# themeshpotato/rust-ray-tracing-in-a-weekend

Measured on AMD Instinct MI355X. Metric: Msamples/s (pixels x spp) for 1200x800 random-spheres scene, higher is better.
Workload: dtype f64

## Files before the change

include/rt/rt_abi.h:

```cpp
#ifndef RT_ABI_H
#define RT_ABI_H

#include <stddef.h>
#include <stdint.h>

#include "rt_scene.h"

#ifdef __cplusplus
extern "C" {
#endif

#define RT_ABI_VERSION 6

enum {
    RT_OK = 0,
    RT_ERR_INVALID = -1,
    RT_ERR_HIP = -2,
    RT_ERR_UNSUPPORTED = -3,
    RT_ERR_OOM = -4,
    RT_ERR_NO_DEVICE = -5,
    RT_ERR_NO_SCENE = -6,
    RT_ERR_COMM = -7,
    RT_ERR_PEER = -8
};
// ... 125 lines not shown
    uint64_t wave_leaf_steps;
    uint64_t camera_lanes;
    uint64_t camera_steps;
    uint64_t shade_lanes;
    uint64_t shade_steps;
    int32_t precision;
    int32_t waves_per_simd;
    int64_t trace_buf_bytes;
    int32_t overlapped;
    int32_t reserved0;
    int64_t ring_bytes;
    int64_t primary_table_bytes;
    double primary_build_ms;
    double primary_walk_share;
    int64_t sky_tiles;
} rt_stats;
int rt_last_stats(rt_ctx* ctx, rt_stats* out);

typedef struct rt_primary_candidates_info {
    int64_t pixels, flagged;
    int64_t candidates;
    int32_t max_candidates;
    int32_t slots;
} rt_primary_candidates_info;
int rt_primary_candidates_host(const rt_scene_soa* scene, const rt_camera* cam, int width, int height, int k_max,
                               uint16_t* records, rt_primary_candidates_info* info);
int rt_primary_sky_tiles_host(const rt_scene_soa* scene, const rt_camera* cam, int width, int height, int k_max,
                              uint8_t* flags, int64_t* count);
int rt_last_counters(rt_ctx* ctx, uint64_t* out, int n);

// ... 308 lines not shown

int rt_ctx_set_variant(rt_ctx* ctx, int slab32, int lds_stack, int lds_nodes);

enum {
    RT_OPT_TRACE_BUF_BYTES = 1,
    RT_OPT_BATCH_OVERLAP = 2,
    RT_OPT_BLOCK_SAMPLES = 3,
    RT_OPT_BLOCK_CHUNKS = 4,
    RT_OPT_EXTRA_FEATURES = 5,
    RT_OPT_HOIST = 6,
    RT_OPT_POOL_RING = 9,
    RT_OPT_COMM_DIRECT = 10,
    RT_OPT_AUTO_DEAL_ORDER = 11,
    RT_OPT_PRIMARY_CANDIDATES = 12,
    RT_OPT_PRIMARY_CANDIDATES_K = 13,
    RT_OPT_SKIP_SKY_TILES = 14
};
int rt_ctx_set_option(rt_ctx* ctx, int key, int64_t value);
int rt_ctx_get_option(rt_ctx* ctx, int key, int64_t* value);

enum { RT_SCHED_CHUNKS = 0, RT_SCHED_POOL = 1, RT_SCHED_ITEMS = 2, RT_SCHED_AUTO = 3 };
int rt_ctx_set_schedule(rt_ctx* ctx, int schedule);

enum { RT_PREC_F64 = 0, RT_PREC_F32 = 1 };
int rt_ctx_set_precision(rt_ctx* ctx, int precision);

int rt_device_eval(rt_ctx* ctx, int fn, const double* x, const double* y, const double* z, double* out, int n);

#ifdef __cplusplus
}
#endif
// ... 2 lines not shown
```

rust-ray-tracing-in-a-weekend_amd/csrc/abi.cpp:

```cpp
#include <hip/hip_runtime.h>

#include <algorithm>
#include <cmath>
#include <cstring>
#include <new>
#include <string>
#include <vector>

#include "rt/rt_abi.h"
#include "rt/rt_numerics.h"
#include "camera_rays.hpp"
#include "ctx_internal.hpp"
#include "deal_cache.hpp"
#include "launch_plan.hpp"
#include "primary_candidates.hpp"
#include "render_internal.hpp"
#include "scene_lower.hpp"
#include "trace_kernel.hpp"

namespace {

thread_local std::string g_last_error;

}
// ... 317 lines not shown
    }
    if (sky) {
        *dealt_tiles = img_tiles - c->sky_n;
        c->stats.sky_tiles = c->sky_n;
    }
    return RT_OK;
}

static int primary_setup(rt_ctx* c, const rt_camera* cam, const rt_render_params* p, const rtp::Plan& pl, bool count_work,
                         hipStream_t stream, rtk::KParams& K, rtk::LaunchOpts& o)
{
    rt_stats& st = c->stats;
    st.primary_table_bytes = 0;
    st.primary_build_ms = 0.0;
    st.primary_walk_share = 0.0;
    const size_t bytes = rtpc::table_bytes(p->width, p->height);
    if (!c->opt_primary || pl.variant != rtk::FEAT_SET_SPHERES || pl.f32 || pl.schedule != RT_SCHED_POOL || !pl.shape.s16 ||
        pl.seed_stage_bytes == 0 || count_work || bytes > rtpc::kMaxTableBytes || p->width < 2 || p->height < 2)
        return RT_OK;
    rtd::Key key = rtd::key_of(c->upload_gen, *cam, *p);
    key.row_begin = 0;
    key.row_stride = key.row_block = 1;
    if (!(c->primary_valid && rtd::same_key(key, c->primary_key) && c->primary_k == c->opt_primary_k)) {
        c->primary_valid = false;
        int rc = c->primary_tab.reserve(stream, bytes + 16);
        if (rc) return rc;
        const size_t n_tiles = (size_t)rtpc::tiles_x_of(p->width) * (size_t)rtpc::tiles_y_of(p->height);
        rc = c->sky_tab.reserve(stream, 16 + n_tiles);
        if (rc) return rc;
        unsigned* const flagged = reinterpret_cast<unsigned*>(c->primary_tab.as<char>() + bytes);
// ... 7 lines not shown
        HIP_TRY(hipMemcpyAsync(&n_sky, c->sky_tab.p, sizeof n_sky, hipMemcpyDeviceToHost, stream));
        HIP_TRY(hipMemcpyAsync(c->sky_flags.data(), c->sky_dev(), n_tiles, hipMemcpyDeviceToHost, stream));
        HIP_TRY(hipStreamSynchronize(stream));
        c->sky_n = (int64_t)n_sky;
        c->sky_gen++;
        float ms = 0.0f;
        HIP_TRY(c->ev_pc.elapsed(0, &ms));
        c->primary_key = key;
        c->primary_k = c->opt_primary_k;
        c->primary_flagged = (int64_t)n_flagged;
        c->primary_valid = true;
        st.primary_build_ms = ms;
    }
    K.primary = c->primary_tab.as<uint4>();
    o.primary = 1;
    st.primary_table_bytes = (int64_t)bytes;
    st.primary_walk_share = (double)c->primary_flagged / ((double)p->width * (double)p->height);
    return RT_OK;
}

static void write_stats(rt_ctx* c, const rtp::Plan& pl, int chunk, int waves_per_simd, bool count)
{
    rt_stats& st = c->stats;
    st.lds_nodes = pl.n_lds_nodes;
    st.variant_features = (int32_t)pl.variant;
    st.slab32 = pl.slab32;
    st.lds_stack = pl.lds_stack;
    st.schedule = pl.schedule;
    st.precision = pl.f32 ? RT_PREC_F32 : RT_PREC_F64;
    st.waves_per_simd = waves_per_simd;
// ... 483 lines not shown
        if (v < 0 || v > 2) return fail(RT_ERR_INVALID, "deal order mode out of range (0 off, 1 auto, 2 measure only)");
        c->opt_deal = (int)v;
        return RT_OK;
    case RT_OPT_PRIMARY_CANDIDATES:
        if (v < 0 || v > 1) return fail(RT_ERR_INVALID, "primary candidates out of range (0 off, 1 on)");
        c->opt_primary = (int)v;
        return RT_OK;
    case RT_OPT_PRIMARY_CANDIDATES_K:
        if (v < 1 || v > rtpc::kSlots) return fail(RT_ERR_INVALID, "primary candidates per pixel out of range (1..7)");
        c->opt_primary_k = (int)v;
        return RT_OK;
    case RT_OPT_SKIP_SKY_TILES:
        if (v < 0 || v > 1) return fail(RT_ERR_INVALID, "skip sky tiles out of range (0 off, 1 on)");
        c->opt_sky = (int)v;
        return RT_OK;
    default: return fail(RT_ERR_INVALID, "unknown option");
    }
}

int rt_ctx_get_option(rt_ctx* c, int key, int64_t* v)
{
    if (!c || !v) return fail(RT_ERR_INVALID, "null argument");
    switch (key) {
    case RT_OPT_TRACE_BUF_BYTES: *v = (int64_t)c->sample_buf_cap; return RT_OK;
    case RT_OPT_BATCH_OVERLAP: *v = c->opt.overlap; return RT_OK;
    case RT_OPT_BLOCK_SAMPLES: *v = c->opt.block_samples; return RT_OK;
    case RT_OPT_BLOCK_CHUNKS: *v = c->opt.block_chunks; return RT_OK;
    case RT_OPT_EXTRA_FEATURES: *v = c->opt.extra_features; return RT_OK;
    case RT_OPT_HOIST: *v = c->opt_hoist; return RT_OK;
    case RT_OPT_POOL_RING: *v = c->opt.ring; return RT_OK;
    case RT_OPT_COMM_DIRECT: *v = c->opt_comm_direct; return RT_OK;
    case RT_OPT_AUTO_DEAL_ORDER: *v = c->opt_deal; return RT_OK;
    case RT_OPT_PRIMARY_CANDIDATES: *v = c->opt_primary; return RT_OK;
    case RT_OPT_PRIMARY_CANDIDATES_K: *v = c->opt_primary_k; return RT_OK;
    case RT_OPT_SKIP_SKY_TILES: *v = c->opt_sky; return RT_OK;
    default: return fail(RT_ERR_INVALID, "unknown option");
    }
}

int rt_ctx_set_schedule(rt_ctx* c, int schedule)
{
    if (c && schedule == 4)
        return fail(RT_ERR_UNSUPPORTED, "schedule 4 (wavefront) was removed: 2.3x slower than the pool on C4 (DESIGN.md 5.7)");
    if (!c || schedule < RT_SCHED_CHUNKS || schedule > RT_SCHED_AUTO) return fail(RT_ERR_INVALID, "bad schedule");
    c->opt.schedule = schedule;
    return RT_OK;
}

int rt_device_eval(rt_ctx* c, int fn, const double* x, const double* y, const double* z, double* out, int n)
{
// ... 19 lines not shown
```

rust-ray-tracing-in-a-weekend_amd/csrc/ctx_internal.hpp:

```cpp
#pragma once

#include <hip/hip_runtime.h>

#include <cstddef>
#include <cstdint>
#include <string>
#include <vector>

#include "rt/rt_abi.h"
#include "deal_cache.hpp"
#include "launch_plan.hpp"
#include "trace_kernel.hpp"

namespace rtx {

int fail(int code, const std::string& msg);
int hip_fail(hipError_t e, const char* what);

}

using rtx::fail;
using rtx::hip_fail;

#define HIP_TRY(expr)                                   \
// ... 147 lines not shown
    DevBuf acc_tmp;
    int opt_deal = rtd::kAuto;
    uint64_t upload_gen = 0;
    rtd::DealCache deal;
    int64_t deal_cap = 0;
    int64_t last_deal_n = 0;
    int opt_primary = 1;
    int opt_primary_k = 7;
    DevBuf primary_tab;
    bool primary_valid = false;
    rtd::Key primary_key;
    int primary_k = 0;
    int64_t primary_flagged = 0;
    EventSpan<2> ev_pc;
    int opt_sky = 1;
    DevBuf sky_tab;
    std::vector<uint8_t> sky_flags;
    int64_t sky_n = 0;
    uint64_t sky_gen = 0;
    uint64_t deal_sky_gen = 0;
    uint8_t* sky_dev() const { return reinterpret_cast<uint8_t*>(sky_tab.p) + 16; }
};

struct StreamScope {
    rt_ctx* c;
    hipStream_t stream;
    bool open = false;
    StreamScope(rt_ctx* c_, hipStream_t s_) : c(c_), stream(s_) {}
    int begin()
    {
// ... 20 lines not shown
```

rust-ray-tracing-in-a-weekend_amd/csrc/trace_kernel.hip:

```cpp
#include "trace_launch.hpp"

namespace rtk {

__device__ __forceinline__ bool tile_slot(SampleTiles g, int n_samples, long long i, long long& px, size_t& rec)
{
    const long long tile = i >> 6;
    const int lp = (int)(i & 63);
    const int x = (int)(tile % g.tiles_x) * 8 + (lp & 7);
    const int k = (int)(tile / g.tiles_x) * 8 + (lp >> 3);
    if (x >= g.width || k >= g.n_rows) return false;
    px = (long long)k * g.width + x;
    rec = tiled_record(g.tiles_x, n_samples, x, k, 0);
    return true;
}

constexpr int kReduceWaves = 8;
template <typename T, typename Rec = double>
__global__ void __launch_bounds__(64 * kReduceWaves) reduce_samples_tiled(const Rec* __restrict__ samples,
                                                                          T* __restrict__ out, SampleTiles g,
                                                                          int n_samples, int chunk, double scale,
                                                                          SkyTiles sky)
{
    __shared__ double part[kReduceWaves][3][64];
    const unsigned tile = blockIdx.x;
// ... 225 lines not shown
}

hipError_t launch_trace(const SceneDev& S, const KParams& Ph, const KParams* P, double* out,
                        unsigned long long* counters, unsigned* work, const LaunchOpts& o, hipStream_t stream)
{
    Launch L;
    L.S = &S;
    L.P = P;
    L.out = out;
    L.counters = counters;
    L.work = work;
    L.pool = o.pool;
    L.waves_per_simd = o.waves_per_simd;
    L.max_waves = o.pool == 1 && Ph.ring ? (unsigned)Ph.ring_waves : 0u;
    L.primary = o.primary != 0 && Ph.primary != nullptr;
    const long long groups = o.pool == 2   ? (Ph.n_chunks + std::max(1, Ph.block_chunks) - 1) / std::max(1, Ph.block_chunks)
                             : o.pool == 1 ? ((long long)Ph.spp - Ph.sample_begin + std::max(1, Ph.block_samples) - 1) /
                                                 std::max(1, Ph.block_samples)
                                           : Ph.n_chunks;
    L.n_blocks = (unsigned long long)Ph.tiles_x * Ph.tiles_y * groups;
    if (L.n_blocks == 0) return hipSuccess;
    if (L.n_blocks > 0xfffffff0ULL) return hipErrorInvalidValue;
    if (o.pool) {
        const hipError_t e = hipMemsetAsync(work, 0, sizeof(unsigned), stream);
        if (e != hipSuccess) return e;
    }
    const uint32_t f = variant_features(o.features);
    if (o.f32) return o.count ? launch_kind<true, true>(f, L, o, stream) : launch_kind<false, true>(f, L, o, stream);
    return o.count ? launch_kind<true, false>(f, L, o, stream) : launch_kind<false, false>(f, L, o, stream);
}
// ... 90 lines not shown
```

rust-ray-tracing-in-a-weekend_amd/csrc/trace_kernel.hpp:

```cpp
#pragma once

#include <hip/hip_runtime.h>

#include "rt/rt_scene.h"
#include "scene_features.hpp"
#include "launch_shapes.hpp"

namespace rtk {

struct SceneDev {
    const rt_prim* prims;
    const int32_t* prim_refs;
    const rt_prim* leaf_prims;
    const rt_bvh_node* nodes;
    const rt_instance* instances;
    const rt_material* materials;
    const rt_texture* textures;
    const double* perlin_ranvec;
    const int32_t* perlin_perm;
    const uint8_t* image;
    int32_t tlas_root;
    int32_t blas_base;
    int32_t stack_entries;
    int32_t n_lds_nodes;
// ... 39 lines not shown
    const uint4* primary;
};

constexpr int32_t kDealOrdered = 2, kDealMeasure = 3;
constexpr unsigned kDealTable = 16;
constexpr bool deal_variant(uint32_t variant) { return variant == FEAT_SET_SPHERES; }

struct LaunchOpts {
    uint32_t features;
    int slab32;
    int lds_stack;
    int count;
    int pool;
    int f32;
    int primary = 0;
    int* waves_per_simd = nullptr;
};

enum CounterSlot : int {
    kCtrCasts = 0,
    kCtrNodeVisits = 1,
    kCtrPrimTests = 2,
    kCtrCyclesCamera = 3,
    kCtrCyclesTrace = 4,
    kCtrCyclesShade = 5,
    kCtrWaveSteps = 6,
    kCtrWaveNodeSteps = 7,
    kCtrCyclesNodes = 8,
    kCtrCyclesLeaves = 9,
    kCtrWaveLeafSteps = 10,
// ... 84 lines not shown
```

rust-ray-tracing-in-a-weekend_amd/csrc/trace_launch.hpp:

```cpp
#pragma once
#include "trace_device.hpp"
#include "trace_launch_common.hpp"

namespace rtk {

template <uint32_t F, bool COUNT, bool F32 = false>
hipError_t launch_variant(const Launch& L, const LaunchOpts& o, hipStream_t stream)
{
    const SceneDev& S = *L.S;
    KernelShape k = launch_shape(F, F32, S, o);
    if constexpr (!F32) {
        if (k.s16) {
            using C = Cfg<F, true, true, true, COUNT, false>;
            static const bool static_lds =
                any_static_lds({(const void*)trace_pool<C, false>, (const void*)trace_pool<C, true>,
                                (const void*)trace_pool<C, false, true>, (const void*)trace_chunks<C>}) ||
                [] {
                    if constexpr (RT_STAGE_SEEDS != 0 && C::SHAPE.s16)
                        return any_static_lds({(const void*)trace_pool<CfgStage<C>, false>, (const void*)trace_pool<CfgStage<C>, false, true>});
                    else return false;
                }() ||
                [] {
                    if constexpr (RT_STAGE_SEEDS != 0 && C::SHAPE.s16 && F == FEAT_SET_SPHERES && !COUNT)
                        return any_static_lds({(const void*)trace_pool<CfgPrimary<C>, false>, (const void*)trace_pool<CfgPrimary<C>, false, true>});
                    else return false;
                }();
            if (static_lds) k = without_stack16(k);
        }
    }
    const int bt = k.block_threads, wpb = bt / 64;
    const int seed_bytes = RT_STAGE_SEEDS && k.s16 && !F32 && L.pool == 1 && S.seed_stage_bytes == (int)seed_stage_bytes_of(bt)
                               ? S.seed_stage_bytes : 0;
    const size_t lds = launch_lds_bytes(k, S, seed_bytes);
    with_cfg<F, COUNT, F32>(k, [&](auto whole, auto part) {
        using C1 = decltype(whole);
        using C0 = decltype(part);
        if (L.pool) {
            auto go = [&](auto kernel) {
                unsigned nb = std::min<unsigned long long>(resident_blocks(L, kernel, lds, bt), (L.n_blocks + wpb - 1) / wpb);
                if (L.max_waves) nb = std::max(1u, std::min(nb, L.max_waves / (unsigned)wpb));
                hipLaunchKernelGGL(kernel, dim3(nb), dim3(bt), lds, stream, S, L.P, L.out, L.counters, L.work);
            };
            if constexpr (RT_STAGE_SEEDS != 0 && C1::SHAPE.s16 && !F32 && F == FEAT_SET_SPHERES && !COUNT) {
                if (seed_bytes && L.primary)
                    return go(L.max_waves ? trace_pool<CfgPrimary<C1>, false, true> : trace_pool<CfgPrimary<C1>, false>);
            }
            if constexpr (RT_STAGE_SEEDS != 0 && C1::SHAPE.s16 && !F32) {
                if (seed_bytes) return go(L.max_waves ? trace_pool<CfgStage<C1>, false, true> : trace_pool<CfgStage<C1>, false>);
            }
            if (L.pool == 2) go(k.nall ? trace_pool<C1, true> : trace_pool<C0, true>);
            else if (L.max_waves)
                go(k.nall ? trace_pool<C1, false, true> : trace_pool<C0, false, true>);
            else go(k.nall ? trace_pool<C1, false> : trace_pool<C0, false>);
            return;
        }
        const auto kernel = k.nall ? trace_chunks<C1> : trace_chunks<C0>;
        if (L.waves_per_simd) (void)blocks_per_cu(L, kernel, lds, bt);
        hipLaunchKernelGGL(kernel, dim3((unsigned)((L.n_blocks + wpb - 1) / wpb)), dim3(bt), lds, stream, S, L.P, L.out, L.counters);
// ... 27 lines not shown
```

rust-ray-tracing-in-a-weekend_amd/csrc/trace_launch_common.hpp:

```cpp
#pragma once
#include "trace_types.hpp"

namespace rtk {

struct Launch {
    const SceneDev* S;
    const KParams* P;
    double* out;
    unsigned long long* counters;
    unsigned* work;
    int pool;
    unsigned long long n_blocks;
    int* waves_per_simd;
    unsigned max_waves = 0;
    bool primary = false;
};

template <class K>
static int blocks_per_cu(const Launch& L, K kernel, size_t lds, int bt)
{
    int per_cu = 0;
    if (hipOccupancyMaxActiveBlocksPerMultiprocessor(&per_cu, kernel, bt, lds) != hipSuccess || per_cu <= 0) per_cu = 1;
    if (L.waves_per_simd) *L.waves_per_simd = per_cu * (bt / 256);
    return per_cu;
}

template <class K>
static unsigned resident_blocks(const Launch& L, K kernel, size_t lds, int bt)
{
    static int cus = 0;
// ... 42 lines not shown
```

rust-ray-tracing-in-a-weekend_amd/csrc/trace_pool.hpp:

```cpp
#pragma once
#include "trace_shade.hpp"
#include "trace_grid.hpp"

namespace rtk {

template <class R>
__device__ __forceinline__ void forget(HitT<R>& h)
{
    h.t = __builtin_nondeterministic_value(h.t);
    h.px = __builtin_nondeterministic_value(h.px);
    h.py = __builtin_nondeterministic_value(h.py);
    h.pz = __builtin_nondeterministic_value(h.pz);
    h.nx = __builtin_nondeterministic_value(h.nx);
    h.ny = __builtin_nondeterministic_value(h.ny);
    h.nz = __builtin_nondeterministic_value(h.nz);
    h.uv0 = __builtin_nondeterministic_value(h.uv0);
    h.uv1 = __builtin_nondeterministic_value(h.uv1);
    h.uv2 = __builtin_nondeterministic_value(h.uv2);
    h.uv3 = __builtin_nondeterministic_value(h.uv3);
    h.front = __builtin_nondeterministic_value(h.front);
    h.mat = __builtin_nondeterministic_value(h.mat);
    h.uvkind = __builtin_nondeterministic_value(h.uvkind);
}

// ... 109 lines not shown
            camera_end(P, st, u, v, qx, qy, r);
            const unsigned n = rec.x & 0xffffu;
            if (n > 7u || depth <= 0) go = true;
            else {
                finish_ray<C, false>(r, true);
                n_cand = n + 1;
            }
        }
        if (__any(n_cand != 0)) {
            const R t_min = (R)0.001;
            R t_max = (R)RT_INF;
            HitRefT<R> best;
            best.sub = 0;
            best.side = 0;
            best.prim = -1;
            uint64_t a = ((uint64_t)rec.y << 32 | (uint64_t)rec.x) >> 16;
            const uint64_t b = (uint64_t)rec.w << 32 | (uint64_t)rec.z;
#pragma unroll 1
            for (unsigned i = 0; __ballot(i + 1 < n_cand) != 0; ++i) {
                if (i + 1 < n_cand) {
                    const int slot = (int)((unsigned)a & 0xffffu);
                    if (simple_t<C>(S.leaf_prims[slot], r, t_min, t_max, best.t, best.side, cnt, false)) {
                        best.prim = slot;
                        t_max = best.t;
                    }
                }
                a >>= 16;
                if (i == 2) a = b;
            }
            if (n_cand != 0) {
                if (best.prim < 0) {
                    cr = cr + Tr * P.bg[0];
                    cg = cg + Tg * P.bg[1];
                    cb = cb + Tb * P.bg[2];
                } else {
                    finish_hit<C>(S, r, best, h);
                    pending = shade_begin<C>(S, h, Tr, Tg, Tb, cr, cg, cb);
                }
            }
        }
    }
    if (__any(pending)) {
        R qx = (R)0, qy = (R)0, qz = (R)0, l2 = (R)1;
        bool accepted = !(pending && shade_draws<C>(S, h.mat));
        for (int n = 1;; ++n) {
            if (!accepted) accepted = unit_try(st, (R)P.scale_m11, true, qx, qy, qz, l2);
            const uint64_t rejecting = __ballot(!accepted);
            if (rejecting == 0 || (n >= RT_TRY_MIN && __popcll(rejecting) <= RT_TRY_LEFT)) break;
        }
        if (pending) {
// ... 460 lines not shown
```

rust-ray-tracing-in-a-weekend_amd/csrc/trace_prims.hpp:

```cpp
#pragma once
#include "trace_types.hpp"

namespace rtk {


template <bool SMALL = false>
__device__ __forceinline__ bool sphere_t(double cx, double cy, double cz, double radius, const RayT<double>& r,
                                         double t_min, double t_max, double& t)
{
    const double ocx = r.ox - cx, ocy = r.oy - cy, ocz = r.oz - cz;
    const double half_b = ocx * r.dx + ocy * r.dy + ocz * r.dz;
    const double c = (ocx * ocx + ocy * ocy + ocz * ocz) - radius * radius;
    const double disc = half_b * half_b - r.a * c;
    if (disc < 0.0) return false;
    const double sqrtd = __builtin_sqrt(disc);
    double root = div_rcp(-half_b - sqrtd, r.a, r.ya);
    if (root < t_min || t_max < root) {
        root = div_rcp(-half_b + sqrtd, r.a, r.ya);
        if (root < t_min || t_max < root) return false;
    }
    t = root;
    return true;
}

__device__ __forceinline__ bool sphere_t2(double cx, double cy, double cz, double radius, const RayT<double>& r,
                                          double& t1, double& t2)
{
    const double ocx = r.ox - cx, ocy = r.oy - cy, ocz = r.oz - cz;
    const double half_b = ocx * r.dx + ocy * r.dy + ocz * r.dz;
    const double c = (ocx * ocx + ocy * ocy + ocz * ocz) - radius * radius;
    const double disc = half_b * half_b - r.a * c;
    if (disc < 0.0) return false;
    const double sqrtd = __builtin_sqrt(disc);
    const double near = div_rcp(-half_b - sqrtd, r.a, r.ya);
// ... 311 lines not shown
```

rust-ray-tracing-in-a-weekend_amd/csrc/trace_types.hpp:

```cpp
#pragma once
#include <hip/hip_runtime.h>

#include <algorithm>
#include <type_traits>

#include "rt/rt_numerics.h"
#include "rt/rt_scene.h"
#include "trace_kernel.hpp"

namespace rtk {

typedef float f2v __attribute__((ext_vector_type(2)));
template <class R>
struct RayT {
    R ox, oy, oz;
    R dx, dy, dz;
    R time;
    R a;
    R ya;
    R ix, iy, iz;
    R yx, yy, yz;
    f2v sx, sy, sz;
    uint32_t onx, ony, onz;
};
// ... 52 lines not shown
template <class C>
constexpr bool TryLeft() { return RT_TRY_LEFT > 0 && (C::F == FEAT_SET_SPHERES || C::F == FEAT_SET_RECTINST); }
template <uint32_t F_, bool S32_, bool LDS_, bool NALL_, bool COUNT_, bool F32_ = false>
struct Cfg {
    static constexpr uint32_t F = F_;
    static constexpr bool S32 = S32_;
    static constexpr bool LDS = LDS_;
    static constexpr bool NALL = NALL_;
    static constexpr bool COUNT = COUNT_;
    static constexpr bool F32 = F32_;
    static constexpr KernelShape SHAPE = kernel_shape(F_, S32_, LDS_, NALL_, F32_);
    static_assert(SHAPE.s32 == S32_ && SHAPE.lds == LDS_ && SHAPE.nall == NALL_ && SHAPE.f32 == F32_, "the shape of this Cfg");
    using Real = typename std::conditional<F32_, float, double>::type;
    static constexpr bool STAGE = false;
    static constexpr bool PRIMARY = false;
};
template <class C>
struct CfgStage : C {
    static constexpr bool STAGE = true;
};

template <class C>
struct CfgPrimary : CfgStage<C> {
    static constexpr bool PRIMARY = true;
};

template <class C>
constexpr int BlockThreads() { return C::SHAPE.block_threads; }

template <class C, uint32_t DROP>
struct CfgDrop : C {
    static constexpr uint32_t F = C::F & ~DROP;
};
template <class C, uint32_t DROP>
struct CfgDropStatic : C {
    static constexpr uint32_t F = (C::F & ~DROP) | ((C::F & FEAT_NEST_MOVING) ? 0u : (uint32_t)FEAT_STATIC);
};
template <class C>
using InstC = CfgDropStatic<C, (C::F & FEAT_INST_RECT) ? 0u : (uint32_t)FEAT_RECT>;
// ... 140 lines not shown
```

rust-ray-tracing-in-a-weekend_amd/csrc/trace_walk.hpp:

```cpp
#pragma once
#include "trace_prims.hpp"

namespace rtk {

constexpr int RT_DONE = (int)0x80000000;

struct Node {
    float lo0[3], hi0[3], lo1[3], hi1[3];
    int child[2];
};
__device__ __forceinline__ Node load_node(const rt_bvh_node* base, int i)
{
    const uint4* q = reinterpret_cast<const uint4*>(base + i);
    const uint4 a = q[0], b = q[1], c = q[2], d = q[3];
    Node n;
    n.lo0[0] = __uint_as_float(a.x); n.lo0[1] = __uint_as_float(a.y); n.lo0[2] = __uint_as_float(a.z);
    n.hi0[0] = __uint_as_float(a.w); n.hi0[1] = __uint_as_float(b.x); n.hi0[2] = __uint_as_float(b.y);
    n.lo1[0] = __uint_as_float(b.z); n.lo1[1] = __uint_as_float(b.w); n.lo1[2] = __uint_as_float(c.x);
    n.hi1[0] = __uint_as_float(c.y); n.hi1[1] = __uint_as_float(c.z); n.hi1[2] = __uint_as_float(c.w);
    n.child[0] = (int)d.x;
    n.child[1] = (int)d.y;
    return n;
}

// ... 30 lines not shown
    return n;
}

template <class C>
constexpr bool StageShade() { return C::SHAPE.stage_shade; }
template <class C>
constexpr bool StageBlas() { return C::SHAPE.stage_blas; }
template <class C>
__device__ __forceinline__ LdsLayout lds_layout_of(const SceneDev& S)
{
    return lds_layout(S.n_lds_nodes, lds_node_bytes<C>(), StageBlas<C>() ? S.n_lds_blas : 0, C::LDS ? S.stack_entries : 0,
                      C::SHAPE.entry_bytes, StageShade<C>() ? S.n_lds_materials : 0,
                      StageShade<C>() ? S.n_lds_textures : 0, BlockThreads<C>());
}

template <class C, bool NL = false, class LeafFn, class R = typename C::Real>
__device__ __forceinline__ bool traverse(const SceneDev& S, int root, const RayT<R>& r, R t_min, R t_max,
                                         HitRefT<R>& best, StackT<C>& stack, int sp0, Count& cnt, LeafFn&& leaf)
{
    const rt_bvh_node* lds_nodes =
        reinterpret_cast<const rt_bvh_node*>(rt_lds);
    bool any = false;
    constexpr int DONE = Stack16Cfg<C>() ? -32768 : RT_DONE;
    constexpr int SSTR = C::LDS ? BlockThreads<C>() : 1;
    auto* sptr = &stack[sp0];
    using SE = typename std::remove_reference<decltype(*sptr)>::type;
    *sptr = (SE)DONE;
    sptr += SSTR;
    auto push = [&](int v) { *sptr = (SE)v; sptr += SSTR; };
    auto pop = [&]() -> int { sptr -= SSTR; return (int)*sptr; };
    int cur = root;
    float tmin_f = 0.0f, tmax_f = 0.0f;
    if constexpr (C::S32) {
        tmin_f = f32_down(t_min);
        tmax_f = f32_up(t_max);
    }
    constexpr bool OCT = NL && OctNodes<C>();
    float ninf = -__builtin_inff();
    if constexpr (OCT) asm("s_mov_b32 %0, 0xff800000" : "=s"(ninf));
    const char* const lb = reinterpret_cast<const char*>(lds_nodes);
    uint32_t blas_lds_base = 0;
    if constexpr (!NL && StageBlas<C>()) blas_lds_base = lds_addr(lb) + (uint32_t)lds_layout_of<C>(S).blas;
    (void)blas_lds_base;
    if constexpr (OCT) cur = cur >= 0 ? (int)(lds_addr(lb) + (uint32_t)cur * (uint32_t)sizeof(LdsNode)) : cur;
    auto visit = [&](int node) -> int {
        if (C::COUNT) cnt.nodes++;
        if constexpr (OCT) {
            const uint32_t nb = (uint32_t)node;
            typedef float f2v __attribute__((ext_vector_type(2)));
            typedef int i2v __attribute__((ext_vector_type(2)));
            auto pairs = [&](uint32_t off, f2v& n, f2v& f) {
// ... 49 lines not shown
        }
        if (h0 && h1) {
            push(near0 ? nd.child[1] : nd.child[0]);
            return near0 ? nd.child[0] : nd.child[1];
        }
        if (h0) return nd.child[0];
        if (h1) return nd.child[1];
        return pop();
    };
    auto do_leaf = [&](int code) {
        code = ~code;
        const int first = code >> 5, count = code & 31;
        for (int i = 0; i < count; ++i) {
            if (C::COUNT && first_active_lane()) cnt.wave_leaves++;
            const int slot = first + i;
            if (leaf(slot, t_max, best)) {
                best.prim = slot;
                t_max = best.t;
                any = true;
                if constexpr (C::S32) tmax_f = f32_up(t_max);
            }
        }
    };
    uint64_t t0 = 0;
    while (cur != DONE) {
        if (C::COUNT && NL) t0 = __builtin_amdgcn_s_memtime();
        while (cur >= 0) {
            if (C::COUNT && first_active_lane()) cnt.wave_nodes++;
            cur = visit(cur);
        }
        if (NL) RT_STAMP(cnt.t_nodes, t0);
        if (cur == DONE) break;
        do_leaf(cur);
        cur = pop();
        if (NL) RT_STAMP(cnt.t_leaves, t0);
    }
    return any;
}

template <class R>
__device__ __forceinline__ void instance_ray(const rt_instance& in, RayT<R>& r)
{
    const int n = in.n_ops;
#pragma unroll
    for (int i = 0; i < 4; ++i) {
        if (i < n) {
            if (in.op_kind[i] == RT_OP_TRANSLATE) {
                r.ox = r.ox - (R)in.op[i][0];
                r.oy = r.oy - (R)in.op[i][1];
                r.oz = r.oz - (R)in.op[i][2];
            } else {
// ... 185 lines not shown
            medium_finish(p, r, best.t, h);
            done = true;
        }
    }
    if (!done) simple_finish<C>(p, r, best.t, best.side, h, (C::F & FEAT_SHUTTER) != 0);
}

template <class C>
constexpr bool PreLeaf() { return C::F == FEAT_SET_SPHERES; }
template <class C>
constexpr bool DeferInst() { return RT_DEFER_INST && (C::F & FEAT_INST_BLAS) != 0; }

template <class C>
constexpr bool UniformLeaf() { return (C::F & FEAT_INST_BLAS) == 0 && !PreLeaf<C>(); }

template <class C, class R = typename C::Real>
__device__ bool trace_world(const SceneDev& S, const RayT<R>& r, HitT<R>& h, StackT<C>& stack, const Keyed& key,
                            Count& cnt)
{
    const R t_min = (R)0.001;
    HitRefT<R> best;
    best.sub = 0;
    best.side = 0;
    int pend = -1;
    (void)pend;
    auto leaf = [&](int slot, R tmax, HitRefT<R>& b) {
        const rt_prim& p = S.leaf_prims[slot];
        if constexpr ((C::F & FEAT_INST) != 0)
            if (p.kind == RT_PRIM_INSTANCE) {
                if constexpr (DeferInst<C>()) {
                    if (pend < 0 && p.b != 0) {
                        pend = slot;
                        return false;
                    }
// ... 93 lines not shown
```

rust-ray-tracing-in-a-weekend_amd/rtiow_amd.py:

```python
from __future__ import annotations

import ctypes
import os
from typing import Optional, Sequence

import numpy as np

HERE = os.path.dirname(os.path.abspath(__file__))
LIB_PATH = os.environ.get("RT_LIB_PATH", os.path.join(HERE, "lib", "librtiow_amd.so"))
REPO = os.path.dirname(HERE)
EARTH_JPG = os.path.join(REPO, "assets", "earthmap.jpg")

RT_OK = 0
ERRORS = {-1: "RT_ERR_INVALID", -2: "RT_ERR_HIP", -3: "RT_ERR_UNSUPPORTED", -4: "RT_ERR_OOM",
          -5: "RT_ERR_NO_DEVICE", -6: "RT_ERR_NO_SCENE", -7: "RT_ERR_COMM", -8: "RT_ERR_PEER"}
RT_COMM_ID_BYTES = 128

SCENES = {"random": 0, "two_spheres": 1, "two_perlin": 2, "earth": 3, "simple_light": 4,
          "cornell": 5, "cornell_smoke": 6, "final": 7}
SCENES_NEEDING_IMAGE = (3, 7)

RT_OUT_F32, RT_OUT_F64 = 0, 1
RT_SCHED_CHUNKS = 0
RT_SCHED_POOL = 1
# ... 4 lines not shown
RT_ACCEL_SAH = 0
RT_ACCEL_LINEAR = 1
RT_ACCEL_MEDIAN = 2
RT_OPT_TRACE_BUF_BYTES = 1
RT_OPT_BATCH_OVERLAP = 2
RT_OPT_BLOCK_SAMPLES = 3
RT_OPT_BLOCK_CHUNKS = 4
RT_OPT_EXTRA_FEATURES = 5
RT_OPT_HOIST = 6
RT_OPT_POOL_RING = 9
RT_OPT_COMM_DIRECT = 10
RT_OPT_AUTO_DEAL_ORDER = 11
RT_OPT_PRIMARY_CANDIDATES = 12
RT_OPT_PRIMARY_CANDIDATES_K = 13
RT_OPT_SKIP_SKY_TILES = 14
RT_BUILD_C_ISECT = 1
RT_BUILD_MAX_LEAF = 2
RT_BUILD_FORCE_LEAF = 3
RT_BUILD_ROOT_LEAF = 4
RT_BUILD_SPLIT_BOX_PAIRS = 5
RT_BUILD_SPLIT_BLAS_PAIRS = 6
RT_BUILD_TIME0 = 7
RT_BUILD_TIME1 = 8

EXPORTED = [
    "rt_abi_version", "rt_last_error", "rt_device_count", "rt_ctx_create", "rt_ctx_destroy",
    "rt_world_create", "rt_world_destroy", "rt_world_texture_solid", "rt_world_texture_checker",
    "rt_world_texture_noise", "rt_world_texture_image", "rt_world_material_lambertian",
    "rt_world_material_metal", "rt_world_material_dielectric", "rt_world_material_diffuse_light",
    "rt_world_material_isotropic", "rt_world_sphere", "rt_world_moving_sphere", "rt_world_rect",
# ... 78 lines not shown
                ("n_items", ctypes.c_uint64), ("n_chunks", ctypes.c_int32), ("spp_chunk", ctypes.c_int32),
                ("scene_bytes", ctypes.c_int64), ("node_bytes", ctypes.c_int32), ("prim_bytes", ctypes.c_int32),
                ("material_bytes", ctypes.c_int32), ("variant_features", ctypes.c_int32),
                ("slab32", ctypes.c_int32), ("lds_stack", ctypes.c_int32), ("lds_nodes", ctypes.c_int32),
                ("cycles_camera", ctypes.c_uint64),
                ("cycles_trace", ctypes.c_uint64), ("cycles_shade", ctypes.c_uint64),
                ("wave_steps", ctypes.c_uint64), ("wave_node_steps", ctypes.c_uint64),
                ("cycles_nodes", ctypes.c_uint64), ("cycles_leaves", ctypes.c_uint64),
                ("schedule", ctypes.c_int32), ("n_batches", ctypes.c_int32),
                ("wave_leaf_steps", ctypes.c_uint64), ("camera_lanes", ctypes.c_uint64),
                ("camera_steps", ctypes.c_uint64), ("shade_lanes", ctypes.c_uint64),
                ("shade_steps", ctypes.c_uint64), ("precision", ctypes.c_int32), ("waves_per_simd", ctypes.c_int32),
                ("trace_buf_bytes", ctypes.c_int64), ("overlapped", ctypes.c_int32), ("reserved0", ctypes.c_int32),
                ("ring_bytes", ctypes.c_int64),
                ("primary_table_bytes", ctypes.c_int64), ("primary_build_ms", ctypes.c_double),
                ("primary_walk_share", ctypes.c_double), ("sky_tiles", ctypes.c_int64)]

    def as_dict(self):
        return {k: getattr(self, k) for k, _ in self._fields_}


class PrimaryCandidatesInfo(ctypes.Structure):
    _fields_ = [("pixels", ctypes.c_int64), ("flagged", ctypes.c_int64), ("candidates", ctypes.c_int64),
                ("max_candidates", ctypes.c_int32), ("slots", ctypes.c_int32)]


class CommStats(ctypes.Structure):
    _fields_ = [("render_ms", ctypes.c_double), ("gather_ms", ctypes.c_double), ("assemble_ms", ctypes.c_double),
                ("kernel_ms", ctypes.c_double), ("slab_bytes", ctypes.c_int64), ("tiles", ctypes.c_int32),
                ("tile_order", ctypes.c_int32), ("cost_pass_ms", ctypes.c_double), ("peer_failed", ctypes.c_int32)]

# ... 1384 lines not shown
```

Baseline: 7664.

## Defer exact f64 sphere roots using f32 interval brackets during traversal

Adds a deferred-root path for the f64 spheres kernel. Each leaf test computes the quadratic in f64 but brackets the root with a conservative f32 interval and its error bound. The exact f64 sqrt and divide run only when two brackets overlap, plus once for the winning primitive before shading. The aim is to drop the costly f64 sqrt and divide from most candidate tests while keeping the same closest hit. It is on by default, adds kernel variants, and depends on the error bound being conservative.

```diff
diff --git a/include/rt/rt_abi.h b/include/rt/rt_abi.h
--- a/include/rt/rt_abi.h
+++ b/include/rt/rt_abi.h
@@ -163,6 +163,7 @@
     double primary_build_ms;
     double primary_walk_share;
     int64_t sky_tiles;
+    int64_t defer_roots;
 } rt_stats;
 int rt_last_stats(rt_ctx* ctx, rt_stats* out);
 
@@ -501,7 +502,8 @@
     RT_OPT_AUTO_DEAL_ORDER = 11,
     RT_OPT_PRIMARY_CANDIDATES = 12,
     RT_OPT_PRIMARY_CANDIDATES_K = 13,
-    RT_OPT_SKIP_SKY_TILES = 14
+    RT_OPT_SKIP_SKY_TILES = 14,
+    RT_OPT_DEFER_ROOTS = 15
 };
 int rt_ctx_set_option(rt_ctx* ctx, int key, int64_t value);
 int rt_ctx_get_option(rt_ctx* ctx, int key, int64_t* value);
diff --git a/rust-ray-tracing-in-a-weekend_amd/csrc/abi.cpp b/rust-ray-tracing-in-a-weekend_amd/csrc/abi.cpp
--- a/rust-ray-tracing-in-a-weekend_amd/csrc/abi.cpp
+++ b/rust-ray-tracing-in-a-weekend_amd/csrc/abi.cpp
@@ -355,6 +355,7 @@
     st.primary_table_bytes = 0;
     st.primary_build_ms = 0.0;
     st.primary_walk_share = 0.0;
+    st.defer_roots = 0;
     const size_t bytes = rtpc::table_bytes(p->width, p->height);
     if (!c->opt_primary || pl.variant != rtk::FEAT_SET_SPHERES || pl.f32 || pl.schedule != RT_SCHED_POOL || !pl.shape.s16 ||
         pl.seed_stage_bytes == 0 || count_work || bytes > rtpc::kMaxTableBytes || p->width < 2 || p->height < 2)
@@ -392,6 +393,8 @@
     }
     K.primary = c->primary_tab.as<uint4>();
     o.primary = 1;
+    o.defer_roots = c->opt_defer_roots;
+    st.defer_roots = c->opt_defer_roots;
     st.primary_table_bytes = (int64_t)bytes;
     st.primary_walk_share = (double)c->primary_flagged / ((double)p->width * (double)p->height);
     return RT_OK;
@@ -905,6 +908,10 @@
         if (v < 0 || v > 1) return fail(RT_ERR_INVALID, "skip sky tiles out of range (0 off, 1 on)");
         c->opt_sky = (int)v;
         return RT_OK;
+    case RT_OPT_DEFER_ROOTS:
+        if (v < 0 || v > 1) return fail(RT_ERR_INVALID, "defer roots out of range (0 off, 1 on)");
+        c->opt_defer_roots = (int)v;
+        return RT_OK;
     default: return fail(RT_ERR_INVALID, "unknown option");
     }
 }
@@ -925,6 +932,7 @@
     case RT_OPT_PRIMARY_CANDIDATES: *v = c->opt_primary; return RT_OK;
     case RT_OPT_PRIMARY_CANDIDATES_K: *v = c->opt_primary_k; return RT_OK;
     case RT_OPT_SKIP_SKY_TILES: *v = c->opt_sky; return RT_OK;
+    case RT_OPT_DEFER_ROOTS: *v = c->opt_defer_roots; return RT_OK;
     default: return fail(RT_ERR_INVALID, "unknown option");
     }
 }
diff --git a/rust-ray-tracing-in-a-weekend_amd/csrc/ctx_internal.hpp b/rust-ray-tracing-in-a-weekend_amd/csrc/ctx_internal.hpp
--- a/rust-ray-tracing-in-a-weekend_amd/csrc/ctx_internal.hpp
+++ b/rust-ray-tracing-in-a-weekend_amd/csrc/ctx_internal.hpp
@@ -185,6 +185,7 @@
     int64_t primary_flagged = 0;
     EventSpan<2> ev_pc;
     int opt_sky = 1;
+    int opt_defer_roots = 1;
     DevBuf sky_tab;
     std::vector<uint8_t> sky_flags;
     int64_t sky_n = 0;
diff --git a/rust-ray-tracing-in-a-weekend_amd/csrc/root_bracket.hpp b/rust-ray-tracing-in-a-weekend_amd/csrc/root_bracket.hpp
--- /dev/null
+++ b/rust-ray-tracing-in-a-weekend_amd/csrc/root_bracket.hpp
@@ -0,0 +1,97 @@
+#pragma once
+
+#include <cstdint>
+
+#ifdef __HIPCC__
+#include <hip/hip_runtime.h>
+#define RT_RB_HD __host__ __device__ inline
+#else
+#define RT_RB_HD inline
+#endif
+
+namespace rtrb {
+
+RT_RB_HD float down(double t)
+{
+    const float f = (float)t;
+    return f > 0.0f ? f * (1.0f - 0x1.0p-20f) : f * (1.0f + 0x1.0p-20f);
+}
+RT_RB_HD float up(double t)
+{
+    const float f = (float)t;
+    return f > 0.0f ? f * (1.0f + 0x1.0p-20f) : f * (1.0f - 0x1.0p-20f);
+}
+
+RT_RB_HD float sqrt32(float x)
+{
+#if defined(__HIP_DEVICE_COMPILE__)
+    return __builtin_amdgcn_sqrtf(x);
+#else
+    return __builtin_sqrtf(x);
+#endif
+}
+
+RT_RB_HD float ya32(double ya)
+{
+    const float y = (float)ya;
+    return y >= 0x1.0p-60f && y <= 0x1.0p+60f ? y : __builtin_nanf("");
+}
+
+RT_RB_HD bool roots(double half_b, double disc, float yaf, float& nlo, float& nhi, float& flo, float& fhi)
+{
+    const float hbf = (float)half_b, df = (float)disc;
+    const float sf = df >= 0x1.0p-80f ? sqrt32(df) : __builtin_nanf("");
+    const float e = ((__builtin_fabsf(hbf) + sf) * yaf) * 0x1.0p-21f;
+    const float tn = (-hbf - sf) * yaf, tf = (sf - hbf) * yaf;
+    nlo = tn - e;
+    nhi = tn + e;
+    flo = tf - e;
+    fhi = tf + e;
+    return e < __builtin_inff();
+}
+
+struct Best {
+    int prim;
+    float lo, hi;
+};
+RT_RB_HD Best none() { return Best{-1, __builtin_inff(), __builtin_inff()}; }
+
+struct Tally {
+    long long bracket = 0, exact = 0;
+};
+
+template <class ExactSelf, class ExactOf>
+RT_RB_HD bool closer(Best& best, int slot, double half_b, double disc, float yaf, float tmin_lo, float tmin_hi,
+                     ExactSelf&& exact_self, ExactOf&& exact_of, Tally* tally = nullptr)
+{
+    float nlo, nhi, flo, fhi;
+    (void)roots(half_b, disc, yaf, nlo, nhi, flo, fhi);
+    const bool use_far = nhi < tmin_lo;
+    const float lo = use_far ? flo : nlo, hi = use_far ? fhi : nhi;
+    const bool behind = fhi < tmin_lo;
+    const bool farther = lo > best.hi;
+    const bool sure = lo >= tmin_hi && hi < best.lo;
+    best.prim = sure ? slot : best.prim;
+    best.lo = sure ? lo : best.lo;
+    best.hi = sure ? hi : best.hi;
+    if (__builtin_expect(behind || farther || sure, 1)) {
+        if (tally) tally->bracket++;
+        return sure;
+    }
+    if (tally) tally->exact++;
+    double t;
+    if (!exact_self(t)) return false;
+    double tb = (double)__builtin_inff();
+    if (best.prim >= 0) (void)exact_of(best.prim, tb);
+    if (tb < t) {
+        best.lo = down(tb);
+        best.hi = up(tb);
+        return false;
+    }
+    best.prim = slot;
+    best.lo = down(t);
+    best.hi = up(t);
+    return true;
+}
+
+}
diff --git a/rust-ray-tracing-in-a-weekend_amd/csrc/trace_kernel.hip b/rust-ray-tracing-in-a-weekend_amd/csrc/trace_kernel.hip
--- a/rust-ray-tracing-in-a-weekend_amd/csrc/trace_kernel.hip
+++ b/rust-ray-tracing-in-a-weekend_amd/csrc/trace_kernel.hip
@@ -263,6 +263,7 @@
     L.waves_per_simd = o.waves_per_simd;
     L.max_waves = o.pool == 1 && Ph.ring ? (unsigned)Ph.ring_waves : 0u;
     L.primary = o.primary != 0 && Ph.primary != nullptr;
+    L.defer_roots = L.primary && o.defer_roots != 0;
     const long long groups = o.pool == 2   ? (Ph.n_chunks + std::max(1, Ph.block_chunks) - 1) / std::max(1, Ph.block_chunks)
                              : o.pool == 1 ? ((long long)Ph.spp - Ph.sample_begin + std::max(1, Ph.block_samples) - 1) /
                                                  std::max(1, Ph.block_samples)
diff --git a/rust-ray-tracing-in-a-weekend_amd/csrc/trace_kernel.hpp b/rust-ray-tracing-in-a-weekend_amd/csrc/trace_kernel.hpp
--- a/rust-ray-tracing-in-a-weekend_amd/csrc/trace_kernel.hpp
+++ b/rust-ray-tracing-in-a-weekend_amd/csrc/trace_kernel.hpp
@@ -77,6 +77,7 @@
     int pool;
     int f32;
     int primary = 0;
+    int defer_roots = 0;
     int* waves_per_simd = nullptr;
 };
 
diff --git a/rust-ray-tracing-in-a-weekend_amd/csrc/trace_launch.hpp b/rust-ray-tracing-in-a-weekend_amd/csrc/trace_launch.hpp
--- a/rust-ray-tracing-in-a-weekend_amd/csrc/trace_launch.hpp
+++ b/rust-ray-tracing-in-a-weekend_amd/csrc/trace_launch.hpp
@@ -24,6 +24,11 @@
                     if constexpr (RT_STAGE_SEEDS != 0 && C::SHAPE.s16 && F == FEAT_SET_SPHERES && !COUNT)
                         return any_static_lds({(const void*)trace_pool<CfgPrimary<C>, false>, (const void*)trace_pool<CfgPrimary<C>, false, true>});
                     else return false;
+                }() ||
+                [] {
+                    if constexpr (RT_STAGE_SEEDS != 0 && C::SHAPE.s16 && F == FEAT_SET_SPHERES && !COUNT)
+                        return any_static_lds({(const void*)trace_pool<CfgDefer<C>, false>, (const void*)trace_pool<CfgDefer<C>, false, true>});
+                    else return false;
                 }();
             if (static_lds) k = without_stack16(k);
         }
@@ -42,6 +47,8 @@
                 hipLaunchKernelGGL(kernel, dim3(nb), dim3(bt), lds, stream, S, L.P, L.out, L.counters, L.work);
             };
             if constexpr (RT_STAGE_SEEDS != 0 && C1::SHAPE.s16 && !F32 && F == FEAT_SET_SPHERES && !COUNT) {
+                if (seed_bytes && L.primary && L.defer_roots)
+                    return go(L.max_waves ? trace_pool<CfgDefer<C1>, false, true> : trace_pool<CfgDefer<C1>, false>);
                 if (seed_bytes && L.primary)
                     return go(L.max_waves ? trace_pool<CfgPrimary<C1>, false, true> : trace_pool<CfgPrimary<C1>, false>);
             }
diff --git a/rust-ray-tracing-in-a-weekend_amd/csrc/trace_launch_common.hpp b/rust-ray-tracing-in-a-weekend_amd/csrc/trace_launch_common.hpp
--- a/rust-ray-tracing-in-a-weekend_amd/csrc/trace_launch_common.hpp
+++ b/rust-ray-tracing-in-a-weekend_amd/csrc/trace_launch_common.hpp
@@ -14,6 +14,7 @@
     int* waves_per_simd;
     unsigned max_waves = 0;
     bool primary = false;
+    bool defer_roots = false;
 };
 
 template <class K>
diff --git a/rust-ray-tracing-in-a-weekend_amd/csrc/trace_pool.hpp b/rust-ray-tracing-in-a-weekend_amd/csrc/trace_pool.hpp
--- a/rust-ray-tracing-in-a-weekend_amd/csrc/trace_pool.hpp
+++ b/rust-ray-tracing-in-a-weekend_amd/csrc/trace_pool.hpp
@@ -147,13 +147,16 @@
             best.sub = 0;
             best.side = 0;
             best.prim = -1;
+            [[maybe_unused]] rtrb::Best bb = rtrb::none();
             uint64_t a = ((uint64_t)rec.y << 32 | (uint64_t)rec.x) >> 16;
             const uint64_t b = (uint64_t)rec.w << 32 | (uint64_t)rec.z;
 #pragma unroll 1
             for (unsigned i = 0; __ballot(i + 1 < n_cand) != 0; ++i) {
                 if (i + 1 < n_cand) {
                     const int slot = (int)((unsigned)a & 0xffffu);
-                    if (simple_t<C>(S.leaf_prims[slot], r, t_min, t_max, best.t, best.side, cnt, false)) {
+                    if constexpr (C::DEFER) {
+                        (void)sphere_defer_t<C>(S, r, rtrb::ya32(r.ya), slot, t_min, bb);
+                    } else if (simple_t<C>(S.leaf_prims[slot], r, t_min, t_max, best.t, best.side, cnt, false)) {
                         best.prim = slot;
                         t_max = best.t;
                     }
@@ -161,12 +164,14 @@
                 a >>= 16;
                 if (i == 2) a = b;
             }
+            if constexpr (C::DEFER) best.prim = bb.prim;
             if (n_cand != 0) {
                 if (best.prim < 0) {
                     cr = cr + Tr * P.bg[0];
                     cg = cg + Tg * P.bg[1];
                     cb = cb + Tb * P.bg[2];
                 } else {
+                    if constexpr (C::DEFER) (void)sphere_exact_of<C>(S, r, best.prim, t_min, best.t);
                     finish_hit<C>(S, r, best, h);
                     pending = shade_begin<C>(S, h, Tr, Tg, Tb, cr, cg, cb);
                 }
diff --git a/rust-ray-tracing-in-a-weekend_amd/csrc/trace_prims.hpp b/rust-ray-tracing-in-a-weekend_amd/csrc/trace_prims.hpp
--- a/rust-ray-tracing-in-a-weekend_amd/csrc/trace_prims.hpp
+++ b/rust-ray-tracing-in-a-weekend_amd/csrc/trace_prims.hpp
@@ -18,6 +18,26 @@
     if (root < t_min || t_max < root) {
         root = div_rcp(-half_b + sqrtd, r.a, r.ya);
         if (root < t_min || t_max < root) return false;
+    }
+    t = root;
+    return true;
+}
+
+__device__ __forceinline__ void sphere_quad(double cx, double cy, double cz, double radius, const RayT<double>& r,
+                                            double& half_b, double& disc)
+{
+    const double ocx = r.ox - cx, ocy = r.oy - cy, ocz = r.oz - cz;
+    half_b = ocx * r.dx + ocy * r.dy + ocz * r.dz;
+    const double c = (ocx * ocx + ocy * ocy + ocz * ocz) - radius * radius;
+    disc = half_b * half_b - r.a * c;
+}
+__device__ __forceinline__ bool sphere_root(double half_b, double disc, const RayT<double>& r, double t_min, double& t)
+{
+    const double sqrtd = __builtin_sqrt(disc);
+    double root = div_rcp(-half_b - sqrtd, r.a, r.ya);
+    if (root < t_min) {
+        root = div_rcp(-half_b + sqrtd, r.a, r.ya);
+        if (root < t_min) return false;
     }
     t = root;
     return true;
diff --git a/rust-ray-tracing-in-a-weekend_amd/csrc/trace_types.hpp b/rust-ray-tracing-in-a-weekend_amd/csrc/trace_types.hpp
--- a/rust-ray-tracing-in-a-weekend_amd/csrc/trace_types.hpp
+++ b/rust-ray-tracing-in-a-weekend_amd/csrc/trace_types.hpp
@@ -90,6 +90,7 @@
     using Real = typename std::conditional<F32_, float, double>::type;
     static constexpr bool STAGE = false;
     static constexpr bool PRIMARY = false;
+    static constexpr bool DEFER = false;
 };
 template <class C>
 struct CfgStage : C {
@@ -99,6 +100,11 @@
 template <class C>
 struct CfgPrimary : CfgStage<C> {
     static constexpr bool PRIMARY = true;
+};
+
+template <class C>
+struct CfgDefer : CfgPrimary<C> {
+    static constexpr bool DEFER = true;
 };
 
 template <class C>
diff --git a/rust-ray-tracing-in-a-weekend_amd/csrc/trace_walk.hpp b/rust-ray-tracing-in-a-weekend_amd/csrc/trace_walk.hpp
--- a/rust-ray-tracing-in-a-weekend_amd/csrc/trace_walk.hpp
+++ b/rust-ray-tracing-in-a-weekend_amd/csrc/trace_walk.hpp
@@ -1,4 +1,5 @@
 #pragma once
+#include "root_bracket.hpp"
 #include "trace_prims.hpp"
 
 namespace rtk {
@@ -68,10 +69,12 @@
                       StageShade<C>() ? S.n_lds_textures : 0, BlockThreads<C>());
 }
 
-template <class C, bool NL = false, class LeafFn, class R = typename C::Real>
+template <class C, bool NL = false, class LeafFn, class R = typename C::Real, class Best = HitRefT<R>>
 __device__ __forceinline__ bool traverse(const SceneDev& S, int root, const RayT<R>& r, R t_min, R t_max,
-                                         HitRefT<R>& best, StackT<C>& stack, int sp0, Count& cnt, LeafFn&& leaf)
-{
+                                         Best& best, StackT<C>& stack, int sp0, Count& cnt, LeafFn&& leaf)
+{
+    constexpr bool DEFER = C::DEFER && NL && std::is_same<Best, rtrb::Best>::value;
+    static_assert(!DEFER || C::S32, "deferred roots: the f32-slab kernels");
     const rt_bvh_node* lds_nodes =
         reinterpret_cast<const rt_bvh_node*>(rt_lds);
     bool any = false;
@@ -89,6 +92,7 @@
         tmin_f = f32_down(t_min);
         tmax_f = f32_up(t_max);
     }
+    if constexpr (DEFER) tmax_f = best.hi;
     constexpr bool OCT = NL && OctNodes<C>();
     float ninf = -__builtin_inff();
     if constexpr (OCT) asm("s_mov_b32 %0, 0xff800000" : "=s"(ninf));
@@ -168,7 +172,9 @@
         for (int i = 0; i < count; ++i) {
             if (C::COUNT && first_active_lane()) cnt.wave_leaves++;
             const int slot = first + i;
-            if (leaf(slot, t_max, best)) {
+            if constexpr (DEFER) {
+                if (leaf(slot, best)) tmax_f = best.hi;
+            } else if (leaf(slot, t_max, best)) {
                 best.prim = slot;
                 t_max = best.t;
                 any = true;
@@ -189,6 +195,7 @@
         cur = pop();
         if (NL) RT_STAMP(cnt.t_leaves, t0);
     }
+    if constexpr (DEFER) return best.prim >= 0;
     return any;
 }
 
@@ -404,10 +411,78 @@
 template <class C>
 constexpr bool UniformLeaf() { return (C::F & FEAT_INST_BLAS) == 0 && !PreLeaf<C>(); }
 
+template <class C>
+__device__ __forceinline__ bool sphere_exact_of(const SceneDev& S, const RayT<double>& r, int slot, double t_min, double& t)
+{
+    static_assert((C::F & FEAT_RECT) == 0 && !C::F32, "deferred roots: the f64 spheres variant");
+    const rt_prim& p = S.leaf_prims[slot];
+    double cx, cy, cz, half_b, disc;
+    sphere_center(p, r, (C::F & FEAT_SHUTTER) != 0, cx, cy, cz, (C::F & FEAT_STATIC) != 0);
+    sphere_quad(cx, cy, cz, p.p[3], r, half_b, disc);
+    if (disc < 0.0) return false;
+    return sphere_root(half_b, disc, r, t_min, t);
+}
+template <class C>
+__device__ __forceinline__ bool sphere_defer_t(const SceneDev& S, const RayT<double>& r, float yaf, int slot, double t_min,
+                                               rtrb::Best& best)
+{
+    static_assert((C::F & FEAT_RECT) == 0 && !C::F32, "deferred roots: the f64 spheres variant");
+    const rt_prim& p = S.leaf_prims[slot];
+    double cx, cy, cz, half_b, disc;
+    sphere_center(p, r, (C::F & FEAT_SHUTTER) != 0, cx, cy, cz, (C::F & FEAT_STATIC) != 0);
+    sphere_quad(cx, cy, cz, p.p[3], r, half_b, disc);
+    if (disc < 0.0) return false;
+    return rtrb::closer(
+        best, slot, half_b, disc, yaf, rtrb::down(t_min), rtrb::up(t_min),
+        [&](double& t) { return sphere_root(half_b, disc, r, t_min, t); },
+        [&](int s, double& t) { return sphere_exact_of<C>(S, r, s, t_min, t); });
+}
+
+template <class C>
+__device__ __forceinline__ bool trace_world_defer(const SceneDev& S, const RayT<double>& r, HitT<double>& h, StackT<C>& stack,
+                                                  Count& cnt)
+{
+    static_assert(PreLeaf<C>() && C::S32 && !C::COUNT, "deferred roots: the f64 spheres variant's timed kernels");
+    const double t_min = 0.001;
+    rtrb::Best best = rtrb::none();
+    const float yaf = rtrb::ya32(r.ya);
+    int root = S.tlas_root;
+    if (S.pre_leaf != 0) {
+        root = S.pre_root;
+        float tn;
+        if (slab32(S.pre_lo, S.pre_hi, r, f32_down(t_min), f32_up(RT_INF), tn)) {
+            const int code = ~S.pre_leaf;
+            double t_max = RT_INF;
+            for (int slot = code >> 5, end = (code >> 5) + (code & 31); slot < end; ++slot) {
+                double t;
+                if (sphere_exact_of<C>(S, r, slot, t_min, t) && !(t_max < t)) {
+                    best.prim = slot;
+                    t_max = t;
+                }
+            }
+            if (best.prim >= 0) {
+                best.lo = f32_down(t_max);
+                best.hi = f32_up(t_max);
+            }
+        }
+    }
+    if (!traverse<C, true>(S, root, r, t_min, RT_INF, best, stack, 0, cnt,
+                           [&](int slot, rtrb::Best& b) { return sphere_defer_t<C>(S, r, yaf, slot, t_min, b); }))
+        return false;
+    HitRefT<double> ref;
+    ref.prim = best.prim;
+    ref.sub = 0;
+    ref.side = 0;
+    (void)sphere_exact_of<C>(S, r, best.prim, t_min, ref.t);
+    finish_hit<C>(S, r, ref, h);
+    return true;
+}
+
 template <class C, class R = typename C::Real>
 __device__ bool trace_world(const SceneDev& S, const RayT<R>& r, HitT<R>& h, StackT<C>& stack, const Keyed& key,
                             Count& cnt)
 {
+    if constexpr (C::DEFER) return trace_world_defer<C>(S, r, h, stack, cnt);
     const R t_min = (R)0.001;
     HitRefT<R> best;
     best.sub = 0;
diff --git a/rust-ray-tracing-in-a-weekend_amd/rtiow_amd.py b/rust-ray-tracing-in-a-weekend_amd/rtiow_amd.py
--- a/rust-ray-tracing-in-a-weekend_amd/rtiow_amd.py
+++ b/rust-ray-tracing-in-a-weekend_amd/rtiow_amd.py
@@ -42,6 +42,7 @@
 RT_OPT_PRIMARY_CANDIDATES = 12
 RT_OPT_PRIMARY_CANDIDATES_K = 13
 RT_OPT_SKIP_SKY_TILES = 14
+RT_OPT_DEFER_ROOTS = 15
 RT_BUILD_C_ISECT = 1
 RT_BUILD_MAX_LEAF = 2
 RT_BUILD_FORCE_LEAF = 3
@@ -150,7 +151,8 @@
                 ("trace_buf_bytes", ctypes.c_int64), ("overlapped", ctypes.c_int32), ("reserved0", ctypes.c_int32),
                 ("ring_bytes", ctypes.c_int64),
                 ("primary_table_bytes", ctypes.c_int64), ("primary_build_ms", ctypes.c_double),
-                ("primary_walk_share", ctypes.c_double), ("sky_tiles", ctypes.c_int64)]
+                ("primary_walk_share", ctypes.c_double), ("sky_tiles", ctypes.c_int64),
+                ("defer_roots", ctypes.c_int64)]
 
     def as_dict(self):
         return {k: getattr(self, k) for k, _ in self._fields_}
```

New measurement: 7779, median of 6. 1.01x the previous value.
